# thu-ml/SageAttention

Measured on AMD Instinct MI355X. Metric: attention TFLOPS (causal, hd=128), kernel-only, as published by the reference, higher is better.
Workload: dtype int8 QK^T + fp8(e4m3) PV, fp32 accumulate

## Files before the change

### include/sage_gfx950.h

```cpp
#ifndef SAGE_GFX950_H
#define SAGE_GFX950_H

#include <stdint.h>

#ifdef __cplusplus
extern "C" {
#endif

#define SAGE_ABI_VERSION 22

#if defined(__GNUC__)
#define SAGE_API __attribute__((visibility("default")))
#else
#define SAGE_API
#endif

#define SAGE_OK 0
#define SAGE_EINVAL (-1)
#define SAGE_ELAUNCH (-2)

#define SAGE_DTYPE_F16 0
#define SAGE_DTYPE_BF16 1

#define SAGE_GRAN_PER_BLOCK 1
#define SAGE_GRAN_PER_WARP 2
#define SAGE_GRAN_PER_THREAD 3
#define SAGE_GRAN_KBLK128 0x100

#define SAGE_QSTYLE_TRITON 0
#define SAGE_QSTYLE_CUDA 1
#define SAGE_QSTYLE_TRITON_THREAD 2

#define SAGE_PV_ACCUM_SINGLE 0
#define SAGE_PV_ACCUM_TWO_LEVEL 1
#define SAGE_PV_ACCUM_TRITON 2

SAGE_API int sage_abi_version(void);
SAGE_API const char *sage_last_error(void);

SAGE_API int sage_work_order(void);
SAGE_API void sage_set_work_order(int group);
SAGE_API int sage_debug_work_order_plan(int nheads, int nqblk, int64_t kv_len, int head_dim, int pv_fp8, int forced, int *group, int *fold, int *left);
SAGE_API int sage_debug_work_item(int bid, int nwg, int nheads, int nqblk, int group, int fold, int left, int *head, int *qrank);

SAGE_API int64_t sage_v_image_bytes(int head_dim, int fp8, int64_t n_kv_tiles_total);

SAGE_API int sage_quant_qk_int8(const void *x, const void *mean, int8_t *out, float *scale,
                       int B, int H, int L, int D,
                       int64_t x_sb, int64_t x_sh, int64_t x_sl,
                       int64_t o_sb, int64_t o_sh, int64_t o_sl,
                       int64_t mean_sb, int64_t mean_sh,
                       int blk, int warp, int gran, int is_key, int style,
                       float pre_scale, int dtype, void *stream);

SAGE_API int sage_varlen_plan_max_seqs(void);
SAGE_API int sage_varlen_plan(const int32_t *cu_seqlens_q, const int32_t *cu_seqlens_k, int nseq, int total_k, int blkq, int blkk,
                              int is_causal, int Hq, int Hkv, int head_dim, int pv_fp8,
                              int32_t *cu_q_scale, int32_t *cu_k_scale, int32_t *seq_order,
                              int32_t *work_items, int work_items_cap, int32_t *slab_first, int32_t *slab_seq, int slab_seq_cap,
                              int32_t *hdr, void *stream);
SAGE_API int sage_debug_varlen_items(const int32_t *lq, const int32_t *lk, int nseq, int is_causal, int Hq, int Hkv, int head_dim, int pv_fp8,
                                     int32_t *items_out, int items_cap, int32_t *hdr_out);

SAGE_API int sage_quant_qk_int8_varlen(const void *x, const void *mean, int8_t *out, float *scale,
                              const int32_t *cu_seqlens, const int32_t *cu_scale,
                              int nseq, int max_seqlen, int H, int D,
                              int64_t x_sl, int64_t x_sh, int64_t o_sl, int64_t o_sh, int64_t mean_sh,
                              int blk, float pre_scale, int dtype, void *stream);

SAGE_API int64_t sage_stats_ws_floats(int B, int H, int L, int D);

SAGE_API int sage_channel_mean(const void *x, void *mean_out, float *ws, int B, int H, int L, int D,
                               int64_t x_sb, int64_t x_sh, int64_t x_sl, int dtype, void *stream);

SAGE_API int sage_prep_v_fp8(const void *v, void *v_image, float *v_scale, float *v_mean, float *ws,
                    int B, int H, int L, int D,
// ... 201 lines not shown
```

### sageattention_amd/_cabi.py

```python
from __future__ import annotations

import ctypes
import os
from ctypes import c_float, c_int, c_int64, c_void_p

_HERE = os.path.dirname(os.path.abspath(__file__))
LIB_PATH = os.environ.get("SAGE_GFX950_LIB") or os.path.join(_HERE, "libsage_gfx950.so")

ABI_VERSION = 22
DTYPE_F16, DTYPE_BF16 = 0, 1
GRAN_PER_BLOCK, GRAN_PER_WARP, GRAN_PER_THREAD = 1, 2, 3
GRAN_KBLK128 = 0x100
QSTYLE_TRITON, QSTYLE_CUDA, QSTYLE_TRITON_THREAD = 0, 1, 2
PV_ACCUM_SINGLE, PV_ACCUM_TWO_LEVEL, PV_ACCUM_TRITON = 0, 1, 2
MASK_BOOL, MASK_F16, MASK_BF16 = 1, 2, 3
ATTR_FP8_EXACT_SCORES, ATTR_FORCE_PERSISTENT, ATTR_FP8_FOLDED_SCORES = 1, 2, 4


class SageLaunchAttr(ctypes.Structure):
    _fields_ = [("struct_bytes", ctypes.c_uint32), ("flags", ctypes.c_uint32), ("launch_ws", c_void_p), ("launch_ws_bytes", c_int64),
                ("grid_out", c_void_p), ("trace", c_void_p), ("trace_wgs", ctypes.c_int32), ("reserved", ctypes.c_int32)]


def launch_attr(launch_ws=None, folded_scores: bool = False, force_persistent: bool = False, grid_out=None, trace=None, trace_wgs: int = 0):
    if launch_ws is None and not folded_scores and grid_out is None and trace is None:
        return None
    a = SageLaunchAttr()
    a.struct_bytes = ctypes.sizeof(SageLaunchAttr)
    a.flags = (ATTR_FP8_FOLDED_SCORES if folded_scores else 0) | (ATTR_FORCE_PERSISTENT if force_persistent else 0)
    if launch_ws is not None:
        a.launch_ws = launch_ws.data_ptr()
        a.launch_ws_bytes = launch_ws.numel() * launch_ws.element_size()
    if grid_out is not None:
        a.grid_out = ctypes.addressof(grid_out)
    if trace is not None:
        a.trace = trace.data_ptr()
        a.trace_wgs = int(trace_wgs)
    a._keep = (launch_ws, grid_out, trace)
    return a


def attr_arg(a):
    return None if a is None else ctypes.byref(a)

_P, _I, _L, _F = c_void_p, c_int, c_int64, c_float
SYMBOLS = {
    "sage_abi_version": (c_int, []),
    "sage_last_error": (ctypes.c_char_p, []),
    "sage_debug_work_order_plan": (c_int, [_I, _I, _L, _I, _I, _I, _P, _P, _P]),
    "sage_debug_work_item": (c_int, [_I, _I, _I, _I, _I, _I, _I, _P, _P]),
    "sage_work_order": (c_int, []),
    "sage_set_work_order": (None, [_I]),
    "sage_v_image_bytes": (c_int64, [_I, _I, _L]),
    "sage_quant_qk_int8": (c_int, [_P, _P, _P, _P, _I, _I, _I, _I, _L, _L, _L, _L, _L, _L, _L, _L,
                                   _I, _I, _I, _I, _I, _F, _I, _P]),
    "sage_quant_qk_int8_varlen": (c_int, [_P, _P, _P, _P, _P, _P, _I, _I, _I, _I, _L, _L, _L, _L, _L,
                                          _I, _F, _I, _P]),
    "sage_stats_ws_floats": (c_int64, [_I, _I, _I, _I]),
    "sage_channel_mean": (c_int, [_P, _P, _P, _I, _I, _I, _I, _L, _L, _L, _I, _P]),
    "sage_channel_mean_varlen": (c_int, [_P, _P, _P, _P, _P, _P, _P, _I, _I, _I, _I, _I, _L, _L, _I, _P]),
    "sage_prep_v_fp8": (c_int, [_P, _P, _P, _P, _P, _I, _I, _I, _I, _L, _L, _L, _F, _I, _P]),
    "sage_prepass_ws_floats": (c_int64, [_I, _I, _I, _I]),
    "sage_prepass_sync_words": (c_int64, [_I, _I]),
    "sage_prepass_max_seqlen": (c_int, []),
    "sage_prepass_max_seqlen_stream": (c_int, [_P]),
    "sage_host_word_alloc": (c_int, [_P, _P]),
    "sage_host_word_free": (c_int, [_P]),
    "sage_prepass_failed_heads": (c_int, [_P, _I, _I, _P]),
    "sage_debug_prepass_fail": (None, [_I]),
    "sage_prepass_kv": (c_int, [_P, _P, _P, _P, _P, _P, _P, _P, _P, _P, _I, _I, _I, _I,
                                _L, _L, _L, _L, _L, _L, _L, _L, _L, _I, _I, _I, _F, _I, _I, _P, _P]),
    "sage_prepass_kv_varlen": (c_int, [_P, _P, _P, _P, _P, _P, _P, _P, _P, _P, _P, _P, _P, _I, _I, _I, _I, _I, _I,
                                       _L, _L, _L, _L, _L, _L, _I, _P, _P]),
    "sage_debug_spin": (c_int, [_I, _I, _P]),
    "sage_prep_v_f16": (c_int, [_P, _P, _P, _I, _I, _I, _I, _L, _L, _L, _I, _P]),
    "sage_prep_v_f16_varlen": (c_int, [_P, _P, _P, _P, _I, _I, _I, _I, _L, _L, _I, _P]),
    "sage_attn_launch_ws_bytes": (c_int64, []),
    "sage_attn_qk_int8_pv_f8": (c_int, [_P, _P, _P, _P, _P, _P, _P, _P, _P, _I, _I, _I, _I, _I, _I,
                                        _L, _L, _L, _L, _L, _L, _L, _L, _L, _I, _I, _I, _F, _I, _I, _P, _P]),
    "sage_attn_qk_int8_pv_f16": (c_int, [_P, _P, _P, _P, _P, _P, _P, _P, _I, _I, _I, _I, _I, _I,
                                         _L, _L, _L, _L, _L, _L, _L, _L, _L, _I, _I, _I, _F, _I, _I, _P, _P]),
    "sage_attn_qk_int8_pv_f16_vrows": (c_int, [_P, _P, _P, _P, _P, _P, _P, _P, _I, _I, _I, _I, _I, _I,
                                               _L, _L, _L, _L, _L, _L, _L, _L, _L, _L, _L, _L, _I, _I, _I, _F, _I, _I, _P, _P]),
# ... 80 lines not shown
```

### sageattention_amd/csrc/sage_attn_kernel.h

```cpp
#pragma once
#include "sage_common.h"
#include "sage_kernels.h"
#include "sage_attn_parts.h"
#include "sage_quant_math.h"
#include "sage_work_order.h"
#include <atomic>
#include <climits>
#include <cstdlib>
#include <type_traits>

#ifndef SAGE_ABL
#define SAGE_ABL 0
#endif
#ifndef SAGE_DIAG_PIPE
#define SAGE_DIAG_PIPE 1
#endif
#ifndef SAGE_KARG_PREFETCH
#define SAGE_KARG_PREFETCH 1
#endif
#ifndef SAGE_TAIL_PIPE
#define SAGE_TAIL_PIPE 1
#endif
#ifndef SAGE_KSEL
#define SAGE_KSEL 1
#endif
#ifndef SAGE_ATTN_TRACE
#define SAGE_ATTN_TRACE 0
#endif

#define SAGE_MIN_WAVES(D, MASK) ((MASK) != 0 ? 2 : ((D) == 64 ? 3 : 2))

#define SAGE_SCALE2_FOLD(d0, d1, s0, s1, c0, c1, m) "v_fma_f32 " d0 ", " s0 ", " c0 ", -" m "\n\tv_fma_f32 " d1 ", " s1 ", " c1 ", -" m "\n\t"
#define SAGE_SCALE2_EXACT(d0, d1, s0, s1, c0, c1, m) "v_add_f32 " d0 ", 0xbe22f983, " s0 "\n\tv_add_f32 " d1 ", 0xbe22f983, " s1 "\n\t" \
                                                      "v_fma_f32 " d0 ", " d0 ", " c0 ", -" m "\n\tv_fma_f32 " d1 ", " d1 ", " c1 ", -" m "\n\t"

#define SAGE_RENAME_S() do { const v4i z4_ = {0, 0, 0, 0};                                                                   \
        asm volatile("s_nop 15\n\ts_nop 7\n\tv_mfma_i32_32x32x32_i8 %0, %2, %2, %3\n\tv_mfma_i32_32x32x32_i8 %1, %2, %2, %4\n\t"     \
                     "s_nop 15\n\ts_nop 7" : "=&v"(sA[0]), "=&v"(sA[1]) : "v"(z4_), "v"(sB[0]), "v"(sB[1])); } while (0)
// ... 833 lines not shown
```

### sageattention_amd/csrc/sage_attn_loop_f8.h

```cpp
#if SAGE_ABL & 2
#define A_NOP_ "s_nop 1\n\t"
#else
#define A_NOP_ ""
#endif
#define A_PV(acc, av, bv)  asm volatile(A_NOP_ "v_mfma_f32_32x32x64_f8f6f4 %0, %1, %2, %0" : "+v"(acc) : "v"(av), "v"(bv))
#define A_QK0(acc, a, b)   asm volatile(A_NOP_ "v_mfma_i32_32x32x32_i8 %0, %1, %2, 0x3e22f983" : "=&v"(acc) : "v"(a), "v"(b))
#define A_QK(acc, a, b)    asm volatile(A_NOP_ "v_mfma_i32_32x32x32_i8 %0, %1, %2, %0" : "+v"(acc) : "v"(a), "v"(b))
#define A_FENCE()          asm volatile("" ::: "memory")
#if SAGE_ABL & 16
#define A_EXP_ "v_mov_b32"
#else
#define A_EXP_ "v_exp_f32"
#endif
            if (it < n_steady || diag_ok || tail_ok) {
                v16i sA[2], sB[2];
                {
                    const unsigned char *ks0 = smem + cur * C::STAGE_BYTES;
                    v4i kf0[2][C::KSTEPS];
#pragma unroll
                    for (int sb = 0; sb < 2; sb++) {
                        const int krow = sb * 32 + n;
#pragma unroll
                        for (int kk = 0; kk < C::KSTEPS; kk++)
                            kf0[sb][kk] = *reinterpret_cast<const v4i *>(ks0 + krow * D + swz_chunk<D>(krow, 2 * kk + g) * 16);
                    }
#pragma unroll
                    for (int kk = 0; kk < C::KSTEPS; kk++)
#pragma unroll
                        for (int sb = 0; sb < 2; sb++)
                            sA[sb] = kk == 0 ? mfma_i8_first(kf0[sb][kk], qf[kk]) : __builtin_amdgcn_mfma_i32_32x32x32_i8(kf0[sb][kk], qf[kk], sA[sb], 0, 0, 0);
                }
                v8i pA = {0, 0, 0, 0, 0, 0, 0, 0}, pB = {0, 0, 0, 0, 0, 0, 0, 0};
                v8i vf[C::DT];
#pragma unroll
                for (int dt = 0; dt < C::DT; dt++) vf[dt] = v8i{0, 0, 0, 0, 0, 0, 0, 0};
                static_assert(KP / 4 == VP / 4 && (KP / 4 == 1 || KP / 4 == 2), "asm LDS-DMA: one or two pieces per wave and image");
                const unsigned lds_base = (unsigned)(size_t)(__attribute__((address_space(3))) unsigned char *)smem;
                const unsigned voff16 = lane * 16;
                const unsigned koff1m = (KP / 4 == 2) ? koff[KP / 4 - 1] - 1024u : 0u;
                const float sm26 = __builtin_ldexpf(p.sm_scale_log2, kSUnitLog2);
                float cs[2];
                cs[0] = sm26 * (qsc * ksc[0][0]);
                cs[1] = KTHREAD ? sm26 * (qsc * ksc[0][1]) : cs[0];
                float alpha_p = 1.0f;
                [[maybe_unused]] int cmy_row_d = 0;
                constexpr int kMaskedScore = (int)0xFF000000;
                auto rescale = [&]() {
                    if ((SAGE_ABL & 1) == 0 && __builtin_amdgcn_ballot_w64(alpha_p != 1.0f) != 0) {
#pragma unroll
                        for (int dt = 0; dt < C::DT; dt++)
#pragma unroll
                            for (int i = 0; i < 16; i++) o[dt][i] *= alpha_p;
                    }
                };
                auto body = [&](auto slot, auto kind, const int n, const int g, v16i (&sc)[2], v16i (&sn)[2], v8i &pp, v8i &pc) {
                    constexpr int KIND = decltype(kind)::value;
                    constexpr bool HAS_DMA = KIND == 0 || KIND == 3, HAS_NEXT = KIND != 2, DIAG = KIND == 1 || KIND == 2;
                    rescale();
                    const int CUR = slot;
                    const int nxt = (CUR + 1 == NSTAGE) ? 0 : CUR + 1, nn = (nxt + 1 == NSTAGE) ? 0 : nxt + 1;
                    const unsigned char *vs = smem + CUR * C::STAGE_BYTES + C::K_TILE_BYTES;
                    const unsigned char *ksn = smem + nxt * C::STAGE_BYTES;
                    if (SAGE_ABL & 32) asm volatile("s_waitcnt lgkmcnt(0)" ::: "memory"); else asm volatile("s_waitcnt vmcnt(0) lgkmcnt(0)" ::: "memory");
                    if ((SAGE_ABL & 4) == 0) __builtin_amdgcn_s_barrier();
                    if constexpr (HAS_DMA) {
                        const unsigned char *ktp = kbase + (long)(it + 2) * KT * p.k_sl - (KIND == 3 ? 1024 : 0);
                        const unsigned char *vtp = vbase + (v_tile0 + (long)(it + 2) * v_tstride) * (long)C::V_IMG_BYTES + wave * (VP / 4) * 1024;
                        const unsigned ldk = lds_base + nn * C::STAGE_BYTES + wave * (KP / 4) * 1024;
                        const unsigned ldv = lds_base + nn * C::STAGE_BYTES + C::K_TILE_BYTES + wave * (VP / 4) * 1024;
                        unsigned keep;
                        unsigned k0 = koff[0], k1m = koff1m;
                        if constexpr (KIND == 3) {
                            const int rmax = Lk - 1 - (it + 2) * KT, l64 = g * 32 + n;
                            const int r0 = ((wave * (KP / 4)) * 64 + l64) / CPR, r1 = ((wave * (KP / 4) + 1) * 64 + l64) / CPR;
                            k0 = k0 + 1024u - (unsigned)((r0 > rmax ? r0 - rmax : 0) * (int)p.k_sl);
                            if constexpr (KP / 4 == 2) k1m = k1m + 1024u - (unsigned)((r1 > rmax ? r1 - rmax : 0) * (int)p.k_sl);
                        }
                        if constexpr (KP / 4 == 2)
                            asm volatile("s_mov_b32 %0, m0\n\ts_mov_b32 m0, %5\n\ts_nop 0\n\t"
                                         "global_load_lds_dwordx4 %1, %3\n\tglobal_load_lds_dwordx4 %2, %3 offset:1024\n\t"
                                         "s_mov_b32 m0, %6\n\ts_nop 0\n\t"
                                         "global_load_lds_dwordx4 %7, %4\n\tglobal_load_lds_dwordx4 %7, %4 offset:1024\n\t"
                                         "s_mov_b32 m0, %0"
                                         : "=&s"(keep) : "v"(k0), "v"(k1m), "s"(ktp), "s"(vtp), "s"(ldk), "s"(ldv), "v"(voff16) : "memory");
                        else
                            asm volatile("s_mov_b32 %0, m0\n\ts_mov_b32 m0, %4\n\ts_nop 0\n\t"
                                         "global_load_lds_dwordx4 %1, %2\n\t"
                                         "s_mov_b32 m0, %5\n\ts_nop 0\n\t"
                                         "global_load_lds_dwordx4 %6, %3\n\t"
                                         "s_mov_b32 m0, %0"
                                         : "=&s"(keep) : "v"(k0), "s"(ktp), "s"(vtp), "s"(ldk), "s"(ldv), "v"(voff16) : "memory");
                    }

                    A_PV(o[0], vf[0], pp);
                    A_FENCE();
                    float ksc_next[NH][2];
                    [[maybe_unused]] float ks4[4];
                    if constexpr (!HAS_NEXT) {
                    } else if constexpr (KTHREAD && SAGE_KSEL) {
                        const long tb = (long)((it + 1) >> p.ks_shift) * ks_tstride;
                        ks4[0] = ks_c[tb]; ks4[1] = ks_c[tb + 1]; ks4[2] = ks_c[tb + 2]; ks4[3] = ks_c[tb + 3];
                    } else load_kscales(it + 1, ksc_next);
                    v4i kfa[C::KSTEPS], kfb[C::KSTEPS];
                    if constexpr (HAS_NEXT) {
#pragma unroll
                        for (int kk = 0; kk < C::KSTEPS; kk++) {
                            kfa[kk] = *reinterpret_cast<const v4i *>(ksn + n * D + swz_chunk<D>(n, 2 * kk + g) * 16);
                        }
                    }
                    A_FENCE();
                    if constexpr (DIAG) {
                        if (CAUSAL ? (crow0 < it * KT + KT - 1) : (Lk < it * KT + KT)) {
                            const int x = (CAUSAL ? cmy_row_d : Lk - 1) - it * KT - 4 * g;
#pragma unroll
                            for (int u = 0; u < 2; u++)
#pragma unroll
                                for (int i = 0; i < 16; i++) sc[u][i] = (u * 32 + 8 * (i >> 2) + (i & 3) <= x) ? sc[u][i] : kMaskedScore;
                        }
                        cs[0] = fmaxf(cs[0], 0x1p-100f);
                        cs[1] = KTHREAD ? fmaxf(cs[1], 0x1p-100f) : cs[0];
                    }
                    int mx0 = INT_MIN, mx1 = INT_MIN;
#pragma unroll
                    for (int u = 0; u < 2; u++)
// ... 63 lines not shown
                    };
                    float ua[4], ub[4];
                    auto g4s = [&](int w, float (&u)[4]) {
                        const int sb = w >> 2, i0 = 4 * (w & 3);
                        if constexpr (SFOLD)
                            asm volatile(SAGE_SCALE2_FOLD("%0", "%1", "%4", "%5", "%8", "%8", "%10") SAGE_SCALE2_FOLD("%2", "%3", "%6", "%7", "%9", "%9", "%11")
                                         : "=&v"(u[0]), "=&v"(u[1]), "=&v"(u[2]), "=&v"(u[3])
                                         : "v"(sc[sb][i0]), "v"(sc[sb][i0 + 1]), "v"(sc[sb][i0 + 2]), "v"(sc[sb][i0 + 3]), "v"(cs[0]), "v"(cs[1]), "v"(mb0), "v"(mb1));
                        else
                            asm volatile("v_add_f32 %0, 0xbe22f983, %4\n\tv_add_f32 %1, 0xbe22f983, %5\n\t"
                                         "v_add_f32 %2, 0xbe22f983, %6\n\tv_add_f32 %3, 0xbe22f983, %7\n\t"
                                         "v_fma_f32 %0, %0, %8, -%10\n\tv_fma_f32 %1, %1, %8, -%10\n\t"
                                         "v_fma_f32 %2, %2, %9, -%11\n\tv_fma_f32 %3, %3, %9, -%11"
                                         : "=&v"(u[0]), "=&v"(u[1]), "=&v"(u[2]), "=&v"(u[3])
                                         : "v"(sc[sb][i0]), "v"(sc[sb][i0 + 1]), "v"(sc[sb][i0 + 2]), "v"(sc[sb][i0 + 3]), "v"(cs[0]), "v"(cs[1]), "v"(mb0), "v"(mb1));
                    };
                    auto g4e = [&](float (&u)[4]) {
                        asm volatile(A_EXP_ " %0, %0\n\t" A_EXP_ " %1, %1\n\t" A_EXP_ " %2, %2\n\t" A_EXP_ " %3, %3" : "+v"(u[0]), "+v"(u[1]), "+v"(u[2]), "+v"(u[3]));
                    };
                    auto g4c = [&](int w, float (&u)[4]) {
                        if (w == 0)
                            asm volatile("v_add_f32 %0, %3, %5\n\tv_add_f32 %1, %4, %6\n\t"
                                         "v_cvt_pk_fp8_f32 %2, %3, %4\n\tv_cvt_pk_fp8_f32 %2, %5, %6 op_sel:[0,0,1]"
                                         : "=&v"(rs0), "=&v"(rs1), "+v"(pc[w]) : "v"(u[0]), "v"(u[1]), "v"(u[2]), "v"(u[3]));
                        else
                            asm volatile("v_add_f32 %0, %0, %3\n\tv_add_f32 %1, %1, %4\n\tv_add_f32 %0, %0, %5\n\tv_add_f32 %1, %1, %6\n\t"
                                         "v_cvt_pk_fp8_f32 %2, %3, %4\n\tv_cvt_pk_fp8_f32 %2, %5, %6 op_sel:[0,0,1]"
                                         : "+v"(rs0), "+v"(rs1), "+v"(pc[w]) : "v"(u[0]), "v"(u[1]), "v"(u[2]), "v"(u[3]));
                    };
                    if constexpr (C::DT == 4) {
                        g4s(0, ua);
                        A_PV(o[2], vf[2], pp);   g4e(ua); g4s(1, ub); g4c(0, ua);
                        A_PV(o[3], vf[3], pp);   g4e(ub); g4s(2, ua); g4c(1, ub);
                        qk_next(0, 0);           g4e(ua); g4s(3, ub); g4c(2, ua);
                        qk_next(0, 1);           g4e(ub); g4s(4, ua); g4c(3, ub);
                        qk_next(0, 2);           g4e(ua);
                        A_FENCE(); read_v(0); read_v(1); A_FENCE();
                        g4s(5, ub); g4c(4, ua);
                        qk_next(0, 3);           g4e(ub); g4s(6, ua); g4c(5, ub);
                        qk_next(1, 0);           g4e(ua); g4s(7, ub); g4c(6, ua);
                        qk_next(1, 1);           g4e(ub);
                        qk_next(1, 2);           g4c(7, ub);
                        qk_next(1, 3);
                        A_FENCE(); read_v(2); read_v(3); A_FENCE();
                    } else {
                        grp(0); grp(1); grp(2); grp(3);
                        qk_next(0, 0); grp(4); grp(5); grp(6);
                        qk_next(0, 1); grp(7); grp(8); grp(9);
                        A_FENCE(); read_v(0); A_FENCE();
                        qk_next(1, 0); grp(10); grp(11); grp(12);
                        qk_next(1, 1);
                        A_FENCE(); read_v(1); A_FENCE();
                        grp(13); grp(14); grp(15);
                    }
                    l_run = l_run * alpha + (rs0 + rs1);
                    if constexpr (!HAS_NEXT) {
                    } else if constexpr (KTHREAD && SAGE_KSEL) {
                        unsigned long long keep;
                        asm volatile("v_mul_f32 %0, %3, %7\n\tv_mul_f32 %1, %4, %7\n\t"
                                     "s_mov_b64 %2, exec\n\ts_mov_b64 exec, %8\n\t"
                                     "v_mul_f32 %0, %5, %7\n\tv_mul_f32 %1, %6, %7\n\t"
                                     "s_mov_b64 exec, %2\n\t"
                                     "v_mul_f32 %0, %9, %0\n\tv_mul_f32 %1, %9, %1"
                                     : "=&v"(cs[0]), "=&v"(cs[1]), "=&s"(keep)
                                     : "s"(ks4[0]), "s"(ks4[1]), "s"(ks4[2]), "s"(ks4[3]), "v"(qsc), "s"(0xFFFFFFFF00000000ull), "v"(sm26));
                    } else {
                        cs[0] = sm26 * (qsc * ksc_next[0][0]);
                        cs[1] = KTHREAD ? sm26 * (qsc * ksc_next[0][1]) : cs[0];
                    }
                    alpha_p = alpha;
                    it++;
                };
                {
                    static_assert(SIX_BODIES, "FP8 PV: both head sizes run the six-body loop");
                    const int left = n_steady - it;
                    int n6 = left / 6, r = left - 6 * n6;
                    SAGE_TSTAMP(8);
                    using I0 = std::integral_constant<int, 0>; using I1 = std::integral_constant<int, 1>; using I2 = std::integral_constant<int, 2>;
#pragma nounroll
                    for (; n6 > 0; n6--) {
                        body(I0{}, I0{}, n, g, sA, sB, pA, pB); body(I1{}, I0{}, n, g, sB, sA, pB, pA); body(I2{}, I0{}, n, g, sA, sB, pA, pB);
                        body(I0{}, I0{}, n, g, sB, sA, pB, pA); body(I1{}, I0{}, n, g, sA, sB, pA, pB); body(I2{}, I0{}, n, g, sB, sA, pB, pA);
                    }
                    SAGE_TSTAMP(13);
                    int lane_r;
                    asm volatile("v_mbcnt_lo_u32_b32 %0, -1, 0\n\tv_mbcnt_hi_u32_b32 %0, -1, %0" : "=v"(lane_r));
                    const int n_r = lane_r & 31, g_r = lane_r >> 5;
#pragma nounroll
                    for (; r > 0; r--) {
                        body(cur, I0{}, n_r, g_r, sA, sB, pA, pB);
                        SAGE_RENAME_S();
                        pA = pB;
                        cur = (cur + 1 == NSTAGE) ? 0 : cur + 1;
                    }
                    SAGE_TSTAMP(14);
                    int lane_t;
                    asm volatile("v_mbcnt_lo_u32_b32 %0, -1, 0\n\tv_mbcnt_hi_u32_b32 %0, -1, %0" : "=v"(lane_t));
                    const int n_t = lane_t & 31, g_t = lane_t >> 5;
                    if constexpr (DIAG_PIPE) {
                        if (diag_ok) {
                            cmy_row_d = row0 - kchunk0 + n_t;
                            body(cur, I1{}, n_t, g_t, sA, sB, pA, pB);
                            cur = (cur + 1 == NSTAGE) ? 0 : cur + 1;
                            body(cur, I2{}, n_t, g_t, sB, sA, pB, pA);
                            cur = (cur + 1 == NSTAGE) ? 0 : cur + 1;
                        }
                    }
                    if constexpr (TAIL_PIPE) {
                        if (tail_ok) {
                            if (SAGE_TAIL_PIPE != 2 && n_iters - it == 3) {
                                body(cur, std::integral_constant<int, 3>{}, n_t, g_t, sA, sB, pA, pB);
                                SAGE_RENAME_S();
                                pA = pB;
                                cur = (cur + 1 == NSTAGE) ? 0 : cur + 1;
                            }
                            body(cur, I1{}, n_t, g_t, sA, sB, pA, pB);
                            cur = (cur + 1 == NSTAGE) ? 0 : cur + 1;
                            body(cur, I2{}, n_t, g_t, sB, sA, pB, pA);
                            cur = (cur + 1 == NSTAGE) ? 0 : cur + 1;
                        }
                    }
                    SAGE_TSTAMP(15);
                    n = n_t;
                    g = g_t;
                }
                rescale();
#pragma unroll
                for (int dt = 0; dt < C::DT; dt++) A_PV(o[dt], vf[dt], pA);
                if (it < n_iters) load_kscales(it, ksc);
                asm volatile("s_nop 15\n\ts_nop 15\n\ts_waitcnt lgkmcnt(0)" : "+v"(sA[0]), "+v"(sA[1])::"memory");
                __builtin_amdgcn_s_barrier();
            }
#undef A_PV
#undef A_QK0
#undef A_QK
#undef A_FENCE
#undef A_NOP_
#undef A_EXP_
```

### sageattention_amd/csrc/sage_cabi.hip

```cpp
#include "../../include/sage_gfx950.h"
#include "sage_common.h"
#include "sage_kernels.h"
#include "sage_work_order.h"

#include <cstdarg>
#include <cstdio>
#include <cstdlib>
#include <cstring>

namespace {

thread_local char g_err[512] = "";

int fail(int code, const char *fmt, ...)
{
    va_list ap;
    va_start(ap, fmt);
    vsnprintf(g_err, sizeof(g_err), fmt, ap);
    va_end(ap);
    return code;
}

inline bool aligned16(const void *p) { return (reinterpret_cast<uintptr_t>(p) & 15u) == 0; }

int check_launch(hipError_t e, const char *what)
{
    if (e != hipSuccess) return fail(SAGE_ELAUNCH, "%s: %s", what, hipGetErrorString(e));
    return SAGE_OK;
}

#define SAGE_REQUIRE(cond, ...) do { if (!(cond)) return fail(SAGE_EINVAL, __VA_ARGS__); } while (0)

struct MaskArg { const void *ptr; int kind; int64_t sb, sh, sq, sk; };

struct LaunchAttr { unsigned *ws; sage::AttnLaunchOpts opts; unsigned *trace; int trace_wgs; };
int read_attr(const SageLaunchAttr *attr, void *stream, bool takes_ws, LaunchAttr &out)
// ... 98 lines not shown
        SAGE_REQUIRE(mask->ptr, "null attn_mask pointer");
        SAGE_REQUIRE(mask->kind >= SAGE_MASK_BOOL && mask->kind <= SAGE_MASK_BF16, "bad mask_kind %d", mask->kind);
        SAGE_REQUIRE(!is_causal, "Mask should be None for causal attention.");
        p.mask = mask->ptr; p.m_sb = mask->sb; p.m_sh = mask->sh; p.m_sq = mask->sq; p.m_sk = mask->sk;
        mask_kind = mask->kind;
    }
    SAGE_REQUIRE(pv_accum >= SAGE_PV_ACCUM_SINGLE && pv_accum <= SAGE_PV_ACCUM_TRITON && (!fp8 || pv_accum != SAGE_PV_ACCUM_TRITON),
                 "bad pv_accum %d", pv_accum);
    const bool two_level = fp8 ? pv_accum == SAGE_PV_ACCUM_TWO_LEVEL : pv_accum == SAGE_PV_ACCUM_TRITON;
    return check_launch(sage::launch_attn(p, D, fp8, is_causal != 0, kthread, two_level, mask_kind, la.opts), "sage_attn launch");
}

}

extern "C" {

SAGE_API int sage_abi_version(void) { return SAGE_ABI_VERSION; }
SAGE_API const char *sage_last_error(void) { return g_err; }
SAGE_API int sage_debug_work_order_plan(int nheads, int nqblk, int64_t kv_len, int head_dim, int pv_fp8, int forced, int *group, int *fold, int *left)
{
    if (nheads <= 0 || nqblk <= 0 || group == nullptr || fold == nullptr || left == nullptr) return fail(SAGE_EINVAL, "sage_debug_work_order_plan: bad argument");
    sage::WorkOrder w;
    const int grid = sage::plan_work_order(w, nheads, nqblk, (long)kv_len, head_dim, pv_fp8 != 0, forced);
    *group = w.group; *fold = w.fold; *left = w.left;
    return grid;
}
SAGE_API int sage_debug_work_item(int bid, int nwg, int nheads, int nqblk, int group, int fold, int left, int *head, int *qrank)
{
    if (head == nullptr || qrank == nullptr || nwg <= 0 || bid < 0 || bid >= nwg || nheads <= 0 || nqblk <= 0 || group < 0 || fold < 0 || fold > 1 ||
        left < 0 || left >= 8 || left > nheads)
        return fail(SAGE_EINVAL, "sage_debug_work_item: bad argument");
    const sage::WorkOrder w = {group, fold, left};
    return sage::work_item(w, bid, nwg, nheads, nqblk, *head, *qrank) ? 1 : 0;
}
SAGE_API int sage_work_order(void) { return sage::work_order(); }
SAGE_API void sage_set_work_order(int group) { sage::set_work_order_mode(group < -1 ? -1 : group); }

SAGE_API int64_t sage_v_image_bytes(int head_dim, int fp8, int64_t n_kv_tiles_total)
{
    return n_kv_tiles_total * (int64_t)head_dim * (fp8 ? 64 : 128);
}

SAGE_API int sage_quant_qk_int8(const void *x, const void *mean, int8_t *out, float *scale,
                       int B, int H, int L, int D,
                       int64_t x_sb, int64_t x_sh, int64_t x_sl,
                       int64_t o_sb, int64_t o_sh, int64_t o_sl,
                       int64_t mean_sb, int64_t mean_sh,
                       int blk, int warp, int gran, int is_key, int style,
                       float pre_scale, int dtype, void *stream)
{
    SAGE_REQUIRE(x && out && scale, "null tensor pointer");
    SAGE_REQUIRE(D == 64 || D == 128, "head_dim must be 64 or 128 (got %d)", D);
    SAGE_REQUIRE(blk == 64 || blk == 128, "blk must be 64 or 128 (got %d)", blk);
    SAGE_REQUIRE(B > 0 && H > 0 && L > 0, "empty tensor");
    SAGE_REQUIRE(dtype == SAGE_DTYPE_F16 || dtype == SAGE_DTYPE_BF16, "bad dtype %d", dtype);
    SAGE_REQUIRE(style >= 0 && style <= 2, "bad style %d", style);
    SAGE_REQUIRE(aligned16(x) && aligned16(out) && (!mean || aligned16(mean)), "x/out/mean must be 16-byte aligned");
    SAGE_REQUIRE(x_sl % 8 == 0 && x_sh % 8 == 0 && x_sb % 8 == 0, "input strides must be multiples of 8 elements");
    SAGE_REQUIRE(o_sl % 16 == 0 && o_sh % 16 == 0 && o_sb % 16 == 0, "int8 output strides must be multiples of 16");
    SAGE_REQUIRE(!mean || (mean_sb % 8 == 0 && mean_sh % 8 == 0), "mean strides must be multiples of 8 elements");
    sage::QuantParams p{};
    p.x = x; p.mean = mean; p.out = out; p.scale = scale; p.cu = nullptr; p.cu_scale = nullptr;
    p.B = B; p.H = H; p.L = L; p.D = D;
    p.x_sb = x_sb; p.x_sh = x_sh; p.x_sl = x_sl; p.o_sb = o_sb; p.o_sh = o_sh; p.o_sl = o_sl;
    p.mean_sb = mean_sb; p.mean_sh = mean_sh;
    p.blk = blk; p.warp = warp; p.style = style; p.dtype = dtype; p.pre_scale = pre_scale;
// ... 859 lines not shown
```

Baseline: 1561.

## Decouple K and V LDS-DMA prefetch distances in the FP8 attention ring

Restructures the three-slot LDS ring so K tiles are prefetched three iterations ahead and V tiles two ahead, issued separately and spread across the body. Waits now use partial vmcnt counts instead of draining all outstanding loads. The aim is to hide more global-memory latency behind the MFMA work and to avoid full vmcnt stalls. It adds peeled prologue and tail bodies for the clamped last K tile, plus a host-side schedule simulator for debugging, which raises the risk of slot-ordering hazards.

```diff
diff --git a/include/sage_gfx950.h b/include/sage_gfx950.h
--- a/include/sage_gfx950.h
+++ b/include/sage_gfx950.h
@@ -42,6 +42,7 @@
 SAGE_API void sage_set_work_order(int group);
 SAGE_API int sage_debug_work_order_plan(int nheads, int nqblk, int64_t kv_len, int head_dim, int pv_fp8, int forced, int *group, int *fold, int *left);
 SAGE_API int sage_debug_work_item(int bid, int nwg, int nheads, int nqblk, int group, int fold, int left, int *head, int *qrank);
+SAGE_API int sage_debug_ring_schedule(int n_steady, int n_iters, int whole_tiles, int last_pair, int ragged_piped, int k_pieces, int v_pieces, int *events, int cap);
 
 SAGE_API int64_t sage_v_image_bytes(int head_dim, int fp8, int64_t n_kv_tiles_total);
 
diff --git a/sageattention_amd/_cabi.py b/sageattention_amd/_cabi.py
--- a/sageattention_amd/_cabi.py
+++ b/sageattention_amd/_cabi.py
@@ -49,6 +49,7 @@
     "sage_last_error": (ctypes.c_char_p, []),
     "sage_debug_work_order_plan": (c_int, [_I, _I, _L, _I, _I, _I, _P, _P, _P]),
     "sage_debug_work_item": (c_int, [_I, _I, _I, _I, _I, _I, _I, _P, _P]),
+    "sage_debug_ring_schedule": (c_int, [_I, _I, _I, _I, _I, _I, _I, _P, _I]),
     "sage_work_order": (c_int, []),
     "sage_set_work_order": (None, [_I]),
     "sage_v_image_bytes": (c_int64, [_I, _I, _L]),
diff --git a/sageattention_amd/csrc/sage_attn_kernel.h b/sageattention_amd/csrc/sage_attn_kernel.h
--- a/sageattention_amd/csrc/sage_attn_kernel.h
+++ b/sageattention_amd/csrc/sage_attn_kernel.h
@@ -4,6 +4,7 @@
 #include "sage_attn_parts.h"
 #include "sage_quant_math.h"
 #include "sage_work_order.h"
+#include "sage_ring_schedule.h"
 #include <atomic>
 #include <climits>
 #include <cstdlib>
diff --git a/sageattention_amd/csrc/sage_attn_loop_f8.h b/sageattention_amd/csrc/sage_attn_loop_f8.h
--- a/sageattention_amd/csrc/sage_attn_loop_f8.h
+++ b/sageattention_amd/csrc/sage_attn_loop_f8.h
@@ -14,6 +14,72 @@
 #endif
             if (it < n_steady || diag_ok || tail_ok) {
                 v16i sA[2], sB[2];
+                static_assert(KP / 4 == VP / 4 && (KP / 4 == 1 || KP / 4 == 2), "asm LDS-DMA: one or two pieces per wave and image");
+                const unsigned lds_base = (unsigned)(size_t)(__attribute__((address_space(3))) unsigned char *)smem;
+                const unsigned voff16 = lane * 16;
+                const unsigned koff1m = (KP / 4 == 2) ? koff[KP / 4 - 1] - 1024u : 0u;
+                auto req_k = [&](auto clamped, const int tile, const int slot, const int n, const int g) {
+                    constexpr bool CLAMP = decltype(clamped)::value;
+                    const unsigned char *ktp = kbase + (long)tile * KT * p.k_sl - (CLAMP ? 1024 : 0);
+                    const unsigned ldk = lds_base + slot * C::STAGE_BYTES + wave * (KP / 4) * 1024;
+                    unsigned keep;
+                    unsigned k0 = koff[0], k1m = koff1m;
+                    if constexpr (CLAMP) {
+                        const int rmax = Lk - 1 - tile * KT, l64 = g * 32 + n;
+                        const int r0 = ((wave * (KP / 4)) * 64 + l64) / CPR, r1 = ((wave * (KP / 4) + 1) * 64 + l64) / CPR;
+                        k0 = k0 + 1024u - (unsigned)((r0 > rmax ? r0 - rmax : 0) * (int)p.k_sl);
+                        if constexpr (KP / 4 == 2) k1m = k1m + 1024u - (unsigned)((r1 > rmax ? r1 - rmax : 0) * (int)p.k_sl);
+                    }
+                    if constexpr (KP / 4 == 2)
+                        asm volatile("s_mov_b32 %0, m0\n\ts_mov_b32 m0, %4\n\ts_nop 0\n\t"
+                                     "global_load_lds_dwordx4 %1, %3\n\tglobal_load_lds_dwordx4 %2, %3 offset:1024\n\t"
+                                     "s_mov_b32 m0, %0"
+                                     : "=&s"(keep) : "v"(k0), "v"(k1m), "s"(ktp), "s"(ldk) : "memory");
+                    else
+                        asm volatile("s_mov_b32 %0, m0\n\ts_mov_b32 m0, %3\n\ts_nop 0\n\t"
+                                     "global_load_lds_dwordx4 %1, %2\n\t"
+                                     "s_mov_b32 m0, %0"
+                                     : "=&s"(keep) : "v"(k0), "s"(ktp), "s"(ldk) : "memory");
+                };
+                auto req_v = [&](const int tile, const int slot) {
+                    const unsigned char *vtp = vbase + (v_tile0 + (long)tile * v_tstride) * (long)C::V_IMG_BYTES + wave * (VP / 4) * 1024;
+                    const unsigned ldv = lds_base + slot * C::STAGE_BYTES + C::K_TILE_BYTES + wave * (VP / 4) * 1024;
+                    unsigned keep;
+                    if constexpr (VP / 4 == 2)
+                        asm volatile("s_mov_b32 %0, m0\n\ts_mov_b32 m0, %3\n\ts_nop 0\n\t"
+                                     "global_load_lds_dwordx4 %1, %2\n\tglobal_load_lds_dwordx4 %1, %2 offset:1024\n\t"
+                                     "s_mov_b32 m0, %0"
+                                     : "=&s"(keep) : "v"(voff16), "s"(vtp), "s"(ldv) : "memory");
+                    else
+                        asm volatile("s_mov_b32 %0, m0\n\ts_mov_b32 m0, %3\n\ts_nop 0\n\t"
+                                     "global_load_lds_dwordx4 %1, %2\n\t"
+                                     "s_mov_b32 m0, %0"
+                                     : "=&s"(keep) : "v"(voff16), "s"(vtp), "s"(ldv) : "memory");
+                };
+                auto req_kv = [&](const int ktile, const int kslot, const int vtile, const int vslot) {
+                    const unsigned char *ktp = kbase + (long)ktile * KT * p.k_sl;
+                    const unsigned char *vtp = vbase + (v_tile0 + (long)vtile * v_tstride) * (long)C::V_IMG_BYTES + wave * (VP / 4) * 1024;
+                    const unsigned ldk = lds_base + kslot * C::STAGE_BYTES + wave * (KP / 4) * 1024;
+                    const unsigned ldv = lds_base + vslot * C::STAGE_BYTES + C::K_TILE_BYTES + wave * (VP / 4) * 1024;
+                    unsigned keep;
+                    if constexpr (KP / 4 == 2)
+                        asm volatile("s_mov_b32 %0, m0\n\ts_mov_b32 m0, %5\n\ts_nop 0\n\t"
+                                     "global_load_lds_dwordx4 %1, %3\n\tglobal_load_lds_dwordx4 %2, %3 offset:1024\n\t"
+                                     "s_mov_b32 m0, %6\n\ts_nop 0\n\t"
+                                     "global_load_lds_dwordx4 %7, %4\n\tglobal_load_lds_dwordx4 %7, %4 offset:1024\n\t"
+                                     "s_mov_b32 m0, %0"
+                                     : "=&s"(keep) : "v"(koff[0]), "v"(koff1m), "s"(ktp), "s"(vtp), "s"(ldk), "s"(ldv), "v"(voff16) : "memory");
+                    else
+                        asm volatile("s_mov_b32 %0, m0\n\ts_mov_b32 m0, %4\n\ts_nop 0\n\t"
+                                     "global_load_lds_dwordx4 %1, %2\n\t"
+                                     "s_mov_b32 m0, %5\n\ts_nop 0\n\t"
+                                     "global_load_lds_dwordx4 %6, %3\n\t"
+                                     "s_mov_b32 m0, %0"
+                                     : "=&s"(keep) : "v"(koff[0]), "s"(ktp), "s"(vtp), "s"(ldk), "s"(ldv), "v"(voff16) : "memory");
+                };
+                const RingPlan ring = ring_plan(n_steady - it, n_iters - it, diag_ok || tail_ok, SAGE_TAIL_PIPE != 2 && tail_ok);
+                if (ring.k_entry == RING_K_WHOLE) req_k(std::false_type{}, ring_k_tile(-1), ring_k_slot(kRingSlots - 1), n, g);
+                else if (ring.k_entry == RING_K_CLAMPED) req_k(std::true_type{}, ring_k_tile(-1), ring_k_slot(kRingSlots - 1), n, g);
                 {
                     const unsigned char *ks0 = smem + cur * C::STAGE_BYTES;
                     v4i kf0[2][C::KSTEPS];
@@ -34,10 +100,6 @@
                 v8i vf[C::DT];
 #pragma unroll
                 for (int dt = 0; dt < C::DT; dt++) vf[dt] = v8i{0, 0, 0, 0, 0, 0, 0, 0};
-                static_assert(KP / 4 == VP / 4 && (KP / 4 == 1 || KP / 4 == 2), "asm LDS-DMA: one or two pieces per wave and image");
-                const unsigned lds_base = (unsigned)(size_t)(__attribute__((address_space(3))) unsigned char *)smem;
-                const unsigned voff16 = lane * 16;
-                const unsigned koff1m = (KP / 4 == 2) ? koff[KP / 4 - 1] - 1024u : 0u;
                 const float sm26 = __builtin_ldexpf(p.sm_scale_log2, kSUnitLog2);
                 float cs[2];
                 cs[0] = sm26 * (qsc * ksc[0][0]);
@@ -53,43 +115,35 @@
                             for (int i = 0; i < 16; i++) o[dt][i] *= alpha_p;
                     }
                 };
+                [[maybe_unused]] bool k_clamped = false;
                 auto body = [&](auto slot, auto kind, const int n, const int g, v16i (&sc)[2], v16i (&sn)[2], v8i &pp, v8i &pc) {
                     constexpr int KIND = decltype(kind)::value;
-                    constexpr bool HAS_DMA = KIND == 0 || KIND == 3, HAS_NEXT = KIND != 2, DIAG = KIND == 1 || KIND == 2;
+                    constexpr int K_REQ = ring_body_k_request(KIND);
+                    constexpr bool V_REQ = ring_body_v_request(KIND), HAS_NEXT = KIND != RING_BODY_LAST, DIAG = KIND == RING_BODY_QK_LAST || KIND == RING_BODY_LAST;
                     rescale();
                     const int CUR = slot;
-                    const int nxt = (CUR + 1 == NSTAGE) ? 0 : CUR + 1, nn = (nxt + 1 == NSTAGE) ? 0 : nxt + 1;
+                    const int nxt = (CUR + 1 == NSTAGE) ? 0 : CUR + 1;
                     const unsigned char *vs = smem + CUR * C::STAGE_BYTES + C::K_TILE_BYTES;
                     const unsigned char *ksn = smem + nxt * C::STAGE_BYTES;
-                    if (SAGE_ABL & 32) asm volatile("s_waitcnt lgkmcnt(0)" ::: "memory"); else asm volatile("s_waitcnt vmcnt(0) lgkmcnt(0)" ::: "memory");
+                    if (SAGE_ABL & 32) asm volatile("s_waitcnt lgkmcnt(0)" ::: "memory");
+                    else asm volatile("s_waitcnt vmcnt(%0) lgkmcnt(0)" ::"n"(ring_body_wait(KIND, KP / 4, VP / 4)) : "memory");
                     if ((SAGE_ABL & 4) == 0) __builtin_amdgcn_s_barrier();
-                    if constexpr (HAS_DMA) {
-                        const unsigned char *ktp = kbase + (long)(it + 2) * KT * p.k_sl - (KIND == 3 ? 1024 : 0);
-                        const unsigned char *vtp = vbase + (v_tile0 + (long)(it + 2) * v_tstride) * (long)C::V_IMG_BYTES + wave * (VP / 4) * 1024;
-                        const unsigned ldk = lds_base + nn * C::STAGE_BYTES + wave * (KP / 4) * 1024;
-                        const unsigned ldv = lds_base + nn * C::STAGE_BYTES + C::K_TILE_BYTES + wave * (VP / 4) * 1024;
-                        unsigned keep;
-                        unsigned k0 = koff[0], k1m = koff1m;
-                        if constexpr (KIND == 3) {
-                            const int rmax = Lk - 1 - (it + 2) * KT, l64 = g * 32 + n;
-                            const int r0 = ((wave * (KP / 4)) * 64 + l64) / CPR, r1 = ((wave * (KP / 4) + 1) * 64 + l64) / CPR;
-                            k0 = k0 + 1024u - (unsigned)((r0 > rmax ? r0 - rmax : 0) * (int)p.k_sl);
-                            if constexpr (KP / 4 == 2) k1m = k1m + 1024u - (unsigned)((r1 > rmax ? r1 - rmax : 0) * (int)p.k_sl);
-                        }
-                        if constexpr (KP / 4 == 2)
-                            asm volatile("s_mov_b32 %0, m0\n\ts_mov_b32 m0, %5\n\ts_nop 0\n\t"
-                                         "global_load_lds_dwordx4 %1, %3\n\tglobal_load_lds_dwordx4 %2, %3 offset:1024\n\t"
-                                         "s_mov_b32 m0, %6\n\ts_nop 0\n\t"
-                                         "global_load_lds_dwordx4 %7, %4\n\tglobal_load_lds_dwordx4 %7, %4 offset:1024\n\t"
-                                         "s_mov_b32 m0, %0"
-                                         : "=&s"(keep) : "v"(k0), "v"(k1m), "s"(ktp), "s"(vtp), "s"(ldk), "s"(ldv), "v"(voff16) : "memory");
-                        else
-                            asm volatile("s_mov_b32 %0, m0\n\ts_mov_b32 m0, %4\n\ts_nop 0\n\t"
-                                         "global_load_lds_dwordx4 %1, %2\n\t"
-                                         "s_mov_b32 m0, %5\n\ts_nop 0\n\t"
-                                         "global_load_lds_dwordx4 %6, %3\n\t"
-                                         "s_mov_b32 m0, %0"
-                                         : "=&s"(keep) : "v"(k0), "s"(ktp), "s"(vtp), "s"(ldk), "s"(ldv), "v"(voff16) : "memory");
+                    const int tile_t = it;
+                    static_assert(ring_body_wait(RING_BODY_KCLAMP_V, KP / 4, VP / 4) == ring_body_wait(RING_BODY_V, KP / 4, VP / 4), "one wait for both");
+                    auto dma_k = [&]() {
+                        if constexpr (KIND == RING_BODY_KV_LAST) {
+                            if (ring_steady_k_request(tile_t, n_steady)) req_k(std::false_type{}, ring_k_tile(tile_t), ring_k_slot(CUR), n, g);
+                        } else if constexpr (K_REQ == RING_K_WHOLE) req_k(std::false_type{}, ring_k_tile(tile_t), ring_k_slot(CUR), n, g);
+                        else if constexpr (KIND == RING_BODY_V && TAIL_PIPE && SAGE_TAIL_PIPE != 2) {
+                            if (k_clamped) req_k(std::true_type{}, ring_k_tile(tile_t), ring_k_slot(CUR), n, g);
+                        }
+                    };
+                    auto dma_v = [&]() {
+                        if constexpr (V_REQ) req_v(ring_v_tile(tile_t), ring_v_slot(CUR));
+                    };
+                    if constexpr (C::DT != 4) {
+                        if constexpr (KIND == RING_BODY_KV) req_kv(ring_k_tile(tile_t), ring_k_slot(CUR), ring_v_tile(tile_t), ring_v_slot(CUR));
+                        else { dma_k(); dma_v(); }
                     }
 
                     A_PV(o[0], vf[0], pp);
@@ -219,12 +273,14 @@
                         g4s(0, ua);
                         A_PV(o[2], vf[2], pp);   g4e(ua); g4s(1, ub); g4c(0, ua);
                         A_PV(o[3], vf[3], pp);   g4e(ub); g4s(2, ua); g4c(1, ub);
+                        dma_k();
                         qk_next(0, 0);           g4e(ua); g4s(3, ub); g4c(2, ua);
                         qk_next(0, 1);           g4e(ub); g4s(4, ua); g4c(3, ub);
                         qk_next(0, 2);           g4e(ua);
                         A_FENCE(); read_v(0); read_v(1); A_FENCE();
                         g4s(5, ub); g4c(4, ua);
                         qk_next(0, 3);           g4e(ub); g4s(6, ua); g4c(5, ub);
+                        dma_v();
                         qk_next(1, 0);           g4e(ua); g4s(7, ub); g4c(6, ua);
                         qk_next(1, 1);           g4e(ub);
                         qk_next(1, 2);           g4c(7, ub);
@@ -260,14 +316,16 @@
                 };
                 {
                     static_assert(SIX_BODIES, "FP8 PV: both head sizes run the six-body loop");
-                    const int left = n_steady - it;
-                    int n6 = left / 6, r = left - 6 * n6;
+                    constexpr bool PEEL = TAIL_PIPE && SAGE_TAIL_PIPE != 2;
+                    using IL = std::integral_constant<int, PEEL ? RING_BODY_KV : RING_BODY_KV_LAST>;
+                    const int n_loop = PEEL ? ring.n_kv : (n_steady > 0 ? n_steady : 0);
+                    int n6 = n_loop / 6, r = n_loop - 6 * n6;
                     SAGE_TSTAMP(8);
                     using I0 = std::integral_constant<int, 0>; using I1 = std::integral_constant<int, 1>; using I2 = std::integral_constant<int, 2>;
 #pragma nounroll
                     for (; n6 > 0; n6--) {
                         body(I0{}, I0{}, n, g, sA, sB, pA, pB); body(I1{}, I0{}, n, g, sB, sA, pB, pA); body(I2{}, I0{}, n, g, sA, sB, pA, pB);
-                        body(I0{}, I0{}, n, g, sB, sA, pB, pA); body(I1{}, I0{}, n, g, sA, sB, pA, pB); body(I2{}, I0{}, n, g, sB, sA, pB, pA);
+                        body(I0{}, I0{}, n, g, sB, sA, pB, pA); body(I1{}, I0{}, n, g, sA, sB, pA, pB); body(I2{}, IL{}, n, g, sB, sA, pB, pA);
                     }
                     SAGE_TSTAMP(13);
                     int lane_r;
@@ -275,7 +333,7 @@
                     const int n_r = lane_r & 31, g_r = lane_r >> 5;
 #pragma nounroll
                     for (; r > 0; r--) {
-                        body(cur, I0{}, n_r, g_r, sA, sB, pA, pB);
+                        body(cur, IL{}, n_r, g_r, sA, sB, pA, pB);
                         SAGE_RENAME_S();
                         pA = pB;
                         cur = (cur + 1 == NSTAGE) ? 0 : cur + 1;
@@ -284,6 +342,14 @@
                     int lane_t;
                     asm volatile("v_mbcnt_lo_u32_b32 %0, -1, 0\n\tv_mbcnt_hi_u32_b32 %0, -1, %0" : "=v"(lane_t));
                     const int n_t = lane_t & 31, g_t = lane_t >> 5;
+#pragma nounroll
+                    for (int i = (PEEL && ring.peeled >= 0) ? 0 : 1; i < 1 + ring.extra_v; i++) {
+                        k_clamped = i == 0 && ring.peeled == RING_BODY_KCLAMP_V;
+                        body(cur, std::integral_constant<int, RING_BODY_V>{}, n_t, g_t, sA, sB, pA, pB);
+                        SAGE_RENAME_S();
+                        pA = pB;
+                        cur = (cur + 1 == NSTAGE) ? 0 : cur + 1;
+                    }
                     if constexpr (DIAG_PIPE) {
                         if (diag_ok) {
                             cmy_row_d = row0 - kchunk0 + n_t;
@@ -295,12 +361,6 @@
                     }
                     if constexpr (TAIL_PIPE) {
                         if (tail_ok) {
-                            if (SAGE_TAIL_PIPE != 2 && n_iters - it == 3) {
-                                body(cur, std::integral_constant<int, 3>{}, n_t, g_t, sA, sB, pA, pB);
-                                SAGE_RENAME_S();
-                                pA = pB;
-                                cur = (cur + 1 == NSTAGE) ? 0 : cur + 1;
-                            }
                             body(cur, I1{}, n_t, g_t, sA, sB, pA, pB);
                             cur = (cur + 1 == NSTAGE) ? 0 : cur + 1;
                             body(cur, I2{}, n_t, g_t, sB, sA, pB, pA);
@@ -315,7 +375,7 @@
 #pragma unroll
                 for (int dt = 0; dt < C::DT; dt++) A_PV(o[dt], vf[dt], pA);
                 if (it < n_iters) load_kscales(it, ksc);
-                asm volatile("s_nop 15\n\ts_nop 15\n\ts_waitcnt lgkmcnt(0)" : "+v"(sA[0]), "+v"(sA[1])::"memory");
+                asm volatile("s_nop 15\n\ts_nop 15\n\ts_waitcnt vmcnt(%2) lgkmcnt(0)" : "+v"(sA[0]), "+v"(sA[1]) : "n"(ring_drain_wait(KP / 4, VP / 4)) : "memory");
                 __builtin_amdgcn_s_barrier();
             }
 #undef A_PV
diff --git a/sageattention_amd/csrc/sage_cabi.hip b/sageattention_amd/csrc/sage_cabi.hip
--- a/sageattention_amd/csrc/sage_cabi.hip
+++ b/sageattention_amd/csrc/sage_cabi.hip
@@ -2,6 +2,7 @@
 #include "sage_common.h"
 #include "sage_kernels.h"
 #include "sage_work_order.h"
+#include "sage_ring_schedule.h"
 
 #include <cstdarg>
 #include <cstdio>
@@ -166,6 +167,13 @@
         return fail(SAGE_EINVAL, "sage_debug_work_item: bad argument");
     const sage::WorkOrder w = {group, fold, left};
     return sage::work_item(w, bid, nwg, nheads, nqblk, *head, *qrank) ? 1 : 0;
+}
+SAGE_API int sage_debug_ring_schedule(int n_steady, int n_iters, int whole_tiles, int last_pair, int ragged_piped, int k_pieces, int v_pieces, int *events, int cap)
+{
+    static_assert(sizeof(sage::RingEvent) == 4 * sizeof(int), "RingEvent is four ints");
+    if (n_iters < 0 || n_steady > n_iters || whole_tiles < 0 || k_pieces <= 0 || v_pieces <= 0 || cap < 0 || (cap > 0 && events == nullptr))
+        return fail(SAGE_EINVAL, "sage_debug_ring_schedule: bad argument");
+    return sage::ring_schedule(n_steady, n_iters, whole_tiles, last_pair != 0, ragged_piped != 0, k_pieces, v_pieces, reinterpret_cast<sage::RingEvent *>(events), cap);
 }
 SAGE_API int sage_work_order(void) { return sage::work_order(); }
 SAGE_API void sage_set_work_order(int group) { sage::set_work_order_mode(group < -1 ? -1 : group); }
diff --git a/sageattention_amd/csrc/sage_ring_schedule.h b/sageattention_amd/csrc/sage_ring_schedule.h
--- /dev/null
+++ b/sageattention_amd/csrc/sage_ring_schedule.h
@@ -0,0 +1,118 @@
+#pragma once
+
+#if defined(__HIPCC__)
+#define SAGE_RING_HD __host__ __device__ __forceinline__
+#else
+#define SAGE_RING_HD inline
+#endif
+
+namespace sage {
+
+constexpr int kRingSlots = 3;
+
+enum : int {
+    RING_BODY_KV = 0,
+    RING_BODY_QK_LAST = 1,
+    RING_BODY_LAST = 2,
+    RING_BODY_KCLAMP_V = 3,
+    RING_BODY_V = 4,
+    RING_BODY_KV_LAST = 5,
+};
+enum : int { RING_K_NONE = 0, RING_K_WHOLE = 1, RING_K_CLAMPED = 2 };
+
+SAGE_RING_HD constexpr int ring_k_tile(int t) { return t + 3; }
+SAGE_RING_HD constexpr int ring_v_tile(int t) { return t + 2; }
+SAGE_RING_HD constexpr int ring_k_slot(int cur) { return cur; }
+SAGE_RING_HD constexpr int ring_v_slot(int cur) { return cur == 0 ? kRingSlots - 1 : cur - 1; }
+
+SAGE_RING_HD constexpr int ring_body_k_request(int kind)
+{
+    return (kind == RING_BODY_KV || kind == RING_BODY_KV_LAST) ? RING_K_WHOLE : kind == RING_BODY_KCLAMP_V ? RING_K_CLAMPED : RING_K_NONE;
+}
+SAGE_RING_HD constexpr bool ring_body_v_request(int kind) { return kind == RING_BODY_KV || kind == RING_BODY_KCLAMP_V || kind == RING_BODY_V || kind == RING_BODY_KV_LAST; }
+SAGE_RING_HD constexpr bool ring_steady_k_request(int t, int n_steady) { return t + 1 < n_steady; }
+SAGE_RING_HD constexpr int ring_body_pieces(int kind, int kp, int vp)
+{
+    return (ring_body_k_request(kind) != RING_K_NONE ? kp : 0) + (ring_body_v_request(kind) ? vp : 0);
+}
+SAGE_RING_HD constexpr int ring_body_wait(int kind, int kp, int vp)
+{
+    return kind == RING_BODY_QK_LAST ? vp : kind == RING_BODY_LAST ? 0 : kp + vp;
+}
+SAGE_RING_HD constexpr int ring_drain_wait(int , int vp) { return vp; }
+
+struct RingPlan {
+    int n_kv;
+    int peeled;
+    int k_entry;
+    int extra_v;
+    int last_pair;
+};
+SAGE_RING_HD RingPlan ring_plan(int n_steady, int n_iters, bool last_pair, bool ragged_piped)
+{
+    const bool tail3 = last_pair && ragged_piped && n_iters - n_steady == 3;
+    RingPlan r;
+    r.n_kv = n_steady > 1 ? n_steady - 1 : 0;
+    r.peeled = n_steady >= 1 ? (tail3 ? RING_BODY_KCLAMP_V : RING_BODY_V) : -1;
+    r.k_entry = n_steady >= 1 ? RING_K_WHOLE : (tail3 ? RING_K_CLAMPED : RING_K_NONE);
+    r.extra_v = tail3 ? 1 : 0;
+    r.last_pair = last_pair ? 1 : 0;
+    return r;
+}
+
+enum : int {
+    RING_EV_REQ_K = 1,
+    RING_EV_REQ_V = 2,
+    RING_EV_WAIT = 3,
+    RING_EV_READ_K = 4,
+    RING_EV_READ_V = 5,
+    RING_EV_BODY = 6,
+};
+struct RingEvent { int op, a, b, c; };
+
+inline int ring_schedule(int n_steady, int n_iters, int whole, bool last_pair, bool ragged_piped, int kp, int vp, RingEvent *ev, int cap)
+{
+    int n = 0;
+    auto put = [&](int op, int a, int b, int c) { if (n < cap) ev[n] = RingEvent{op, a, b, c}; n++; };
+    auto req_tile = [&](int tile, int slot) {
+        put(RING_EV_REQ_K, tile, slot, tile < whole ? RING_K_WHOLE : RING_K_CLAMPED);
+        put(RING_EV_REQ_V, tile, slot, 0);
+    };
+    if (n_iters > 0) req_tile(0, 0);
+    if (n_iters > 1) req_tile(1, 1);
+    put(RING_EV_WAIT, n_iters > 1 ? kp + vp : 0, 0, 0);
+    int it = 0, cur = 0;
+    if (0 < n_steady || last_pair) {
+        const RingPlan pl = ring_plan(n_steady, n_iters, last_pair, ragged_piped);
+        if (pl.k_entry != RING_K_NONE) put(RING_EV_REQ_K, 2, 2, pl.k_entry);
+        put(RING_EV_READ_K, 0, 0, 0);
+        auto body = [&](int kind) {
+            put(RING_EV_BODY, it, kind, cur);
+            put(RING_EV_WAIT, ring_body_wait(kind, kp, vp), 0, 0);
+            if (ring_body_k_request(kind) != RING_K_NONE) put(RING_EV_REQ_K, ring_k_tile(it), ring_k_slot(cur), ring_body_k_request(kind));
+            if (ring_body_v_request(kind)) put(RING_EV_REQ_V, ring_v_tile(it), ring_v_slot(cur), 0);
+            if (kind != RING_BODY_LAST) put(RING_EV_READ_K, it + 1, (cur + 1) % kRingSlots, 0);
+            put(RING_EV_READ_V, it, cur, 0);
+            it++;
+            cur = (cur + 1) % kRingSlots;
+        };
+        for (int i = 0; i < n_steady; i++) body(ring_steady_k_request(i, n_steady) ? RING_BODY_KV : pl.peeled);
+        if (pl.last_pair) {
+            if (pl.extra_v) body(RING_BODY_V);
+            body(RING_BODY_QK_LAST);
+            body(RING_BODY_LAST);
+        }
+        put(RING_EV_WAIT, ring_drain_wait(kp, vp), 0, 0);
+    }
+    for (; it < n_iters; it++) {
+        put(RING_EV_BODY, it, -1, cur);
+        if (it + 2 < n_iters) req_tile(it + 2, (cur + 2) % kRingSlots);
+        put(RING_EV_READ_K, it, cur, 0);
+        put(RING_EV_READ_V, it, cur, 0);
+        put(RING_EV_WAIT, it + 2 < n_iters ? kp + vp : 0, 0, 0);
+        cur = (cur + 1) % kRingSlots;
+    }
+    return n;
+}
+
+}
```

Result: no change. 1557 (-0.2%).
